# kekeliu-whu/Wildcat-SLAM

Measured on AMD Instinct MI355X. Metric: surfel-extract Mpts/s, higher is better.
Workload: dtype f64; 1 GPU; C2: 1M-pt single scan (G2 patch lattice, 999936 pts -> 31248 surfels) per GPU, voxel-grid + 3-level octree + per-cell 3x3 PCA; input = the reference's 48-byte hilti_ros::Point records, consumed in place; points_per_gpu=999936, surfels_per_gpu=31248, parallelism=sweep-per-gpu x1

## Files before the change

### wildcat-slam_amd/csrc/ctx.h

```cpp
#pragma once
#include <hip/hip_runtime.h>

#include <cstdarg>
#include <cstdio>
#include <cstdlib>
#include <cstring>
#include <string>
#include <vector>

#include "../../include/wildcat_hip.h"

struct wc_window_state;

struct wc_buf {
  void *p = nullptr;
  size_t cap = 0;
  bool pooled = false;
  bool plain = false;
};

#ifdef WC_DEV_KNOBS
#define WC_DBG(P, bit) ((P).dbg & (bit))
#else
#define WC_DBG(P, bit) 0
#endif

struct wc_dev_opts {
  int exact_sums = 0;
  int debug_skip = 0;
  int fx_merge_min = 3;
  int fx_split = -1;
  int no_bucket_sort = 0;
  int ex_sync = 0;
  int match_pair_serial = 0;
  int lm_dense = 0;
  int lm_side_stream = 1;
  int lm_one_collective = 0;
  int map_mom_pts = 1;
  int map_lin_groups = 0;
  int lm_dense_radius = 7;
  int lm_radius0 = -1;
};
inline bool wc_log_env(const char *name) { return getenv(name) != nullptr; }

struct wc_ctx {
  int device = 0;
// ... 37 lines not shown
    int general_calls = 0;
    bool bucket_attr_set = false;
    uint32_t lds_cap = 256;
    bool unordered = false;
    uint32_t last_splits = 256;
    uint32_t ticket = 0, ticket_seq = 0;
    bool fx_active = false;
    bool fx_dirty = false;
    uint32_t fx_last_flags = 0, fx_fallbacks = 0, fx_last_why = 0;
    bool fx_spill_full = false;
    bool fx_split = false;
    bool batch_defer = false, deferred = false;
    unsigned fx_tiles = 0, fx_ngrid = 0;
    bool fx_long_lists = false;
    bool fx_long_lists2 = false;
    uint32_t fx_backoff = 0, fx_skip_calls = 0;
    bool fx_ctrl_ready = false;
    int fx_parity = 0;
    bool precleared = false;
    bool layer2_done = true;
    int (*tail)(wc_ctx *, bool) = nullptr;
    alignas(16) unsigned char roots_args[768];
    uint64_t total_slots;
    uint32_t bin_cap;
    unsigned slot_end_bit;
    bool fast_slots;
  } ex;
  wc_window_state *win = nullptr;
  wc_ctx *aux = nullptr;
  hipEvent_t ev_aux = nullptr;
// ... 74 lines not shown
```

### wildcat-slam_amd/csrc/ctx.hip

```cpp
#include "ctx.h"

#include <cmath>
#include <cstring>
#include <mutex>

extern "C" const char *wc_version(void) { return "wildcat_hip 0.1 (gfx950)"; }

extern "C" int wc_device_count(void) {
  int n = 0;
  if (hipGetDeviceCount(&n) != hipSuccess) return 0;
  return n;
}

extern "C" void wc_params_default(wc_params *p) {
  std::memset(p, 0, sizeof(*p));
  p->voxel_size = 0.8f;
  p->max_layer = 2;
  p->min_points = 20;
  p->planer_threshold = 0.01f;
  p->min_plane_likeness = 0.1;
  p->cluster_gap = 0.05;
  p->cluster_min_points = 20;
  p->center_scale = 1.0;
  p->angular_scale = 5.0 * M_PI / 180.0;
// ... 22 lines not shown
  if (p->knn_k < 1 || p->knn_k > 16) return wc_fail(ctx, WC_ERR_ARG, "knn_k must be 1..16");
  return WC_OK;
}

namespace {
struct DevOpt {
  const char *name, *env;
  int wc_dev_opts::*field;
  bool flag_only;
};
const DevOpt kDevOpts[] = {
    {"exact_sums", "WC_EXACT_SUMS", &wc_dev_opts::exact_sums, true},
    {"debug_skip", "WC_DEBUG_SKIP", &wc_dev_opts::debug_skip, false},
    {"fx_merge_min", "WC_FX_MERGE_MIN", &wc_dev_opts::fx_merge_min, false},
    {"fx_split", "WC_FX_SPLIT", &wc_dev_opts::fx_split, false},
    {"no_bucket_sort", "WC_NO_BUCKET_SORT", &wc_dev_opts::no_bucket_sort, true},
    {"ex_sync", "WC_EX_SYNC", &wc_dev_opts::ex_sync, true},
    {"match_pair_serial", "WC_MATCH_PAIR_SERIAL", &wc_dev_opts::match_pair_serial, true},
    {"lm_dense", "WC_LM_DENSE", &wc_dev_opts::lm_dense, true},
    {"lm_one_collective", "WC_LM_ONE_COLLECTIVE", &wc_dev_opts::lm_one_collective, true},
    {"lm_side_stream", "WC_LM_SIDE_STREAM", &wc_dev_opts::lm_side_stream, false},
    {"map_mom_pts", "WC_MAP_MOM_PTS", &wc_dev_opts::map_mom_pts, false},
    {"map_lin_groups", "WC_MAP_LIN_GROUPS", &wc_dev_opts::map_lin_groups, false},
    {"lm_dense_radius", "WC_LM_DENSE_RADIUS", &wc_dev_opts::lm_dense_radius, false},
    {"lm_radius0", "WC_LM_RADIUS0", &wc_dev_opts::lm_radius0, false},
};
}

namespace {
struct DevPool {
// ... 318 lines not shown
```

### wildcat-slam_amd/csrc/extract.hip

```cpp
#include <hip/hip_runtime.h>
#include <type_traits>

#include <chrono>
#include <cstdlib>
#include <cstring>
#include <rocprim/rocprim.hpp>

#include "ctx.h"
#include "dmath.h"

namespace {

constexpr int kMom = 11;
constexpr int kProdStride = 66;
constexpr unsigned kRootsGrid = 256 * 16;
constexpr unsigned kEmitGrid = 256 * 8;
constexpr unsigned kRoots2Grid = 256 * 4;
constexpr int kBuckets = 4096;
constexpr int kTile = 2048;
constexpr uint32_t kFlagKeyRange = 1u, kFlagSlotOverflow = 2u, kFlagTimeRange = 4u, kFlagBucketOverflow = 8u, kFlagSlotBinOverflow = 16u, kFlagLdsOverflow = 32u;

struct ExParams {
  double vs;
  float vs_f;
// ... 1238 lines not shown
  for (int off = 32; off >= 1; off >>= 1) part += __shfl_xor(part, off);
  if (lane == 0) s_red[w] = part;
  __syncthreads();
  uint32_t base = s_red[0] + s_red[1] + s_red[2] + s_red[3];
  const uint32_t c0 = own.x, c1 = own.y, c2 = own.z, c3 = own.w;
  if (bid == nblk - 1 && t == 0) {
    status[0] = base + c0 + c1 + c2 + c3;
    uint32_t *hm = host_mailbox(status);
    if (hm) {
      hm[0] = base + c0 + c1 + c2 + c3;
      uint32_t queued = status[4];
      const uint32_t *fxc = counts + kBuckets;
      for (int j = 0; j < 16; ++j) queued += fxc[(16 + j) * 32];
      hm[4] = queued;
      hm[5] = status[5];
    }
  }
  base += (w > 0 ? c0 : 0u) + (w > 1 ? c1 : 0u) + (w > 2 ? c2 : 0u);
  const uint32_t c = w == 0 ? c0 : (w == 1 ? c1 : (w == 2 ? c2 : c3));
  if (c == 0) return;
  if (c > bin_cap) {
    if (lane == 0) raise_flag(status, kFlagSlotBinOverflow);
    return;
  }
  auto before = [&](uint64_t other, uint64_t mine) -> bool {
    if ((other >> 32) == (mine >> 32) && other != mine) {
      const double to = slots[(uint32_t)other].t, tm = slots[(uint32_t)mine].t;
      return to < tm || (to == tm && surfel_id_less(slot_ids[(uint32_t)other], slot_ids[(uint32_t)mine]));
    }
    return other < mine;
// ... 333 lines not shown
}

template <typename K>
int sort_pairs(wc_ctx *ctx, K *kin, K *kout, uint32_t *vin, uint32_t *vout, size_t n, unsigned end_bit) {
  using cfg = rocprim::radix_sort_config<rocprim::default_config, rocprim::default_config, rocprim::default_config, 0>;
  size_t tmp = 0;
  WC_HIP(ctx, rocprim::radix_sort_pairs<cfg>(nullptr, tmp, kin, kout, vin, vout, n, 0u, end_bit, ctx->stream));
  WC_TRY(wc_ensure(ctx, ctx->b_sorttmp, tmp));
  tmp = ctx->b_sorttmp.cap;
  WC_HIP(ctx, rocprim::radix_sort_pairs<cfg>(ctx->b_sorttmp.p, tmp, kin, kout, vin, vout, n, 0u, end_bit, ctx->stream));
  return WC_OK;
}

#include "extract_fast.inc"
#include "extract_split.inc"

int fx_ensure_zero(wc_ctx *ctx, wc_buf &b, size_t bytes) {
  if (bytes <= b.cap) return WC_OK;
  WC_TRY(wc_ensure(ctx, b, bytes));
  WC_HIP(ctx, hipMemsetAsync(b.p, 0, b.cap, ctx->stream));
  return WC_OK;
}

bool fx_applicable(const wc_ctx *ctx, uint64_t n, double t_lo, double t_hi) {
  const wc_params &P = ctx->P;
  if (P.exact_sums || ctx->dev.exact_sums) return false;
  if (n < 64 || !(P.voxel_size > 0.0f) || P.voxel_size >= 0.99f) return false;
  if (!(P.cluster_gap > 1e-6) || !(t_hi > t_lo)) return false;
  if ((t_hi - t_lo) / (P.cluster_gap * 0.999) >= 1048000.0) return false;
  return true;
// ... 28 lines not shown
  A.inv_vs = 1.0 / (double)P.voxel_size;
  A.qs = 4294967296.0, A.inv_q = 1.0 / 4294967296.0, A.inv_qq = std::ldexp(1.0, -44);
  uint32_t mr = 1024;
  while ((uint64_t)mr * 8 < n) mr *= 2;
  A.mr_per = mr / kFxSub, A.mq_per = std::max(64u, mr / 2 / kFxSub);
  uint32_t tr = 2048;
  while ((uint64_t)tr * 4 < n) tr *= 2;
  A.tr_mask = tr - 1;
  A.static_map = n <= 2000000ull ? 1u : 0u;
  {
    const uintptr_t px = (uintptr_t)pts.xyz, pt = (uintptr_t)pts.time;
    if (pts.xyz_stride == 48u && pts.time_stride == 48u && pt == px + 24u && px % 16u == 0u)
      A.fmt = 1u;
    else if (pts.xyz_stride == 12u && pts.time_stride == 8u && px % 16u == 0u && pt % 16u == 0u)
      A.fmt = 2u;
  }
  const unsigned tiles = (unsigned)((n + kFxTile - 1) / kFxTile);
  A.rec_tiles = tiles;
  const uint64_t spill_full = ((uint64_t)tiles + 7) / 8 * kFxTile;
  A.spill_per = (uint32_t)((n <= 8000000ull || ctx->ex.fx_spill_full) ? spill_full : std::max<uint64_t>(1024, n / 32));
  A.rec_cap = tiles * (uint32_t)kFxRecTile + 8u * A.spill_per;
  const uint64_t total_slots = std::max<uint64_t>((n * (uint64_t)(P.max_layer + 1)) / (uint64_t)P.cluster_min_points + 1, (uint64_t)kFxSub * 256);
  uint32_t bin_cap = 64;
  while (bin_cap < kSlotBinMax && (uint64_t)bin_cap * kBuckets < 2 * total_slots) bin_cap *= 2;
  WC_TRY(fx_ensure_zero(ctx, ctx->b_fx[0], (size_t)tr * 4));
  WC_TRY(wc_ensure(ctx, ctx->b_fx[1], (size_t)mr * 4));
  WC_TRY(fx_ensure_zero(ctx, ctx->b_fx[2], (size_t)tr * kFxBlockW * 8));
  WC_TRY(fx_ensure_zero(ctx, ctx->b_fx[3], (size_t)A.mq_per * kFxSub * kFxBlockW * 8));
  WC_TRY(wc_ensure(ctx, ctx->b_fx[4], (size_t)2 * A.rec_cap * kFxRecW * 8));
  const unsigned ngrid = std::min<unsigned>(256 * 16, std::max<unsigned>(64, (unsigned)(n / 256)));
// ... 59 lines not shown
  };
  if (dbg) fprintf(stderr, "[fx] n=%llu tiles=%u mr_per=%u mq_per=%u tr=%u slots_per=%u bin_cap=%u\n", (unsigned long long)n, tiles, A.mr_per, A.mq_per, tr, A.slots_per, bin_cap);
  if (ctx->ex.batch_defer) {
    static_assert(sizeof(FxArgs) <= sizeof(ctx->ex.roots_args), "ctx.h: roots_args too small");
    std::memcpy(ctx->ex.roots_args, &A, sizeof(A));
    ctx->ex.total_slots = total_slots;
    ctx->ex.bin_cap = bin_cap;
    ctx->ex.fast_slots = true;
    ctx->ex.tail = &fx_tail;
    ctx->ex.d_out = d_out, ctx->ex.d_ids = d_ids, ctx->ex.cap = cap;
    ctx->ex.layer2_done = P.max_layer >= 2 && ctx->ex.last_splits > 0;
    ctx->ex.fx_tiles = tiles, ctx->ex.fx_ngrid = std::max(64u, ngrid / 8u);
    ctx->ex.deferred = true;
    return WC_OK;
  }
  k_fx_acc<1><<<tiles, kFxThreads, 0, st>>>(A);
  dbg_sync("k_fx_acc<1>");
  mark(2);
  if (ctx->ex.fx_long_lists) k_fx_merge<1><<<std::min<unsigned>(ngrid * 2u, 8192u), 128, 0, st>>>(A);
  if (ctx->ex.fx_split) {
    k_fx_walk<1><<<ngrid, 64, 0, st>>>(A);
    dbg_sync("k_fx_walk<1>");
    k_fx_test<1><<<ngrid, 64, 0, st>>>(A);
  } else {
    k_fx_nodes<1><<<ngrid, 64, 0, st>>>(A);
  }
  dbg_sync("k_fx_nodes<1>");
  mark(3);
  static_assert(sizeof(FxArgs) <= sizeof(ctx->ex.roots_args), "ctx.h: roots_args too small");
  std::memcpy(ctx->ex.roots_args, &A, sizeof(A));
  ctx->ex.total_slots = total_slots;
// ... 6 lines not shown

constexpr int kMailTicket = 120;
__global__ void k_ex_ticket(uint32_t *host_word, uint32_t ticket) {
  __hip_atomic_store(host_word, ticket, __ATOMIC_RELEASE, __HIP_MEMORY_SCOPE_SYSTEM);
}

int fx_tail(wc_ctx *ctx, bool layer2) {
  hipStream_t st = ctx->stream;
  FxArgs A;
  std::memcpy(&A, ctx->ex.roots_args, sizeof(A));
  auto mark = [&](int i) {
    if (ctx->ex_prof && (ctx->ex_prof_mode != 2 || i == 1 || i == 5)) (void)hipEventRecord(ctx->ex_ev[i], st);
  };
  if (layer2) {
    const unsigned tiles = (unsigned)((A.pts.n + kFxTile - 1) / kFxTile);
    k_fx_acc<2><<<tiles, kFxThreads, 0, st>>>(A);
    const unsigned ngrid = std::min<unsigned>(256 * 16, std::max<unsigned>(64, (unsigned)(A.pts.n / 256)));
    if (ctx->ex.fx_long_lists2) k_fx_merge<2><<<std::min(8192u, std::max(64u, ctx->ex.last_splits)), 128, 0, st>>>(A);
    const unsigned g2 = std::min(std::min(256u * 8u, ngrid), std::max(64u, ctx->ex.last_splits));
    if (ctx->ex.fx_split) {
      k_fx_walk<2><<<g2, 64, 0, st>>>(A);
      k_fx_test<2><<<g2, 64, 0, st>>>(A);
    } else {
      k_fx_nodes<2><<<g2, 64, 0, st>>>(A);
    }
  }
  ctx->ex.layer2_done = layer2;
  mark(4);
  uint32_t *next_ctrl = (uint32_t *)ctx->b_fx[5].p + (size_t)(ctx->ex.fx_parity ^ 1) * kCtrlWords;
  static_assert(kCtrlWords <= (kBuckets / 4) * 256, "k_slot_emit's grid covers the control block");
  k_slot_emit<<<kBuckets / 4, 256, 0, st>>>(A.slot_counts, A.slot_bins, ctx->ex.bin_cap, (const wc_surfel *)ctx->b_slots.p,
// ... 291 lines not shown
      for (int i = 0; i < 24; ++i)
        if (ctx->h_status[32 + i]) ctx->ex.fx_last_why |= 1u << i;
      if (ctx->ex.fx_last_why & (1u << 4)) ctx->ex.fx_spill_full = true;
      ctx->ex.fx_backoff = std::min(32u, std::max(1u, ctx->ex.fx_backoff * 2u));
      ctx->ex.fx_skip_calls = ctx->ex.fx_backoff - 1u;
      ctx->ex.fx_dirty = true;
      ctx->ex.fx_ctrl_ready = false;
      ctx->ex.fx_active = false;
      ctx->ex.general = ctx->ex.general_calls > 0;
      WC_TRY(run_pipeline<uint32_t>(ctx, ctx->ex.pts, ctx->ex.t_lo, ctx->ex.t_hi, ctx->ex.d_out, ctx->ex.d_ids, ctx->ex.cap, !ctx->ex.general, true));
      WC_TRY(wait());
    } else {
      const uint32_t n_fast = ctx->h_status[0];
      ctx->ex.fx_long_lists = ctx->h_status[15] != 0u;
      ctx->ex.fx_long_lists2 = ctx->h_status[16] != 0u;
      if (h_n_out) *h_n_out = n_fast;
      ctx->ex.fx_parity ^= 1;
      ctx->ex.fx_backoff = 0;
      if (n_fast > ctx->ex.cap)
        return wc_fail(ctx, WC_ERR_CAPACITY, "output capacity %llu < %u surfels", (unsigned long long)ctx->ex.cap, n_fast);
      return WC_OK;
    }
  }
  while ((ctx->h_status[1] & kFlagLdsOverflow) && !(ctx->h_status[1] & (kFlagBucketOverflow | kFlagKeyRange)) && !ctx->ex.general &&
         ctx->ex.lds_cap < kPtBinMax) {
    ctx->ex.lds_cap *= 2;
    WC_TRY(run_pipeline<uint32_t>(ctx, ctx->ex.pts, ctx->ex.t_lo, ctx->ex.t_hi, ctx->ex.d_out, ctx->ex.d_ids, ctx->ex.cap, true, true));
    WC_TRY(wait());
  }
  if ((ctx->h_status[1] & kFlagLdsOverflow) && !ctx->ex.general) ctx->h_status[1] |= kFlagBucketOverflow;
// ... 54 lines not shown
  hipStream_t st = ctx->stream;
  std::vector<FxArgs> args;
  std::vector<SlotEmitArgs> emit;
  std::vector<uint32_t> s_acc(1, 0u), s_nodes(1, 0u), s_g2(1, 0u), flags;
  bool any_l2 = false, any_merge = false;
  for (int k = 0; k < K; ++k) {
    wc_ctx *sub = ctx->batch_subs[k];
    if (sub->stream != st) WC_TRY(wc_ctx_set_stream(sub, st));
    if (std::memcmp(&sub->P, &ctx->P, sizeof(wc_params)) != 0) WC_TRY(wc_ctx_set_params(sub, &ctx->P));
    if (std::memcmp(&sub->dev, &ctx->dev, sizeof(wc_dev_opts)) != 0) {
      sub->dev = ctx->dev;
      sub->ex.fx_backoff = sub->ex.fx_skip_calls = 0;
    }
    sub->ex.batch_defer = true;
    sub->ex.deferred = false;
    const int rc = wc_extract_surfels_enqueue(sub, &jobs[k].pts, jobs[k].t_lo, jobs[k].t_hi, jobs[k].d_out, jobs[k].d_ids, jobs[k].cap);
    sub->ex.batch_defer = false;
    if (rc != WC_OK) {
      for (int j = 0; j <= k; ++j) {
        wc_ctx *pj = ctx->batch_subs[j];
        if (pj->ex.deferred || j == k) pj->ex.fx_dirty = true, pj->ex.active = false, pj->ex.deferred = false;
      }
      return wc_fail(ctx, rc, "wc_extract_surfels_batch (sweep %d): %s", k, wc_last_error(sub));
    }
    if (!sub->ex.deferred) continue;
    FxArgs A;
    std::memcpy(&A, sub->ex.roots_args, sizeof(A));
    args.push_back(A);
    const uint32_t g2 = std::min(std::min(256u * 8u, sub->ex.fx_ngrid), std::max(64u, sub->ex.last_splits));
    s_acc.push_back(s_acc.back() + sub->ex.fx_tiles);
// ... 15 lines not shown
  std::memcpy(host.data(), args.data(), sizeof(FxArgs) * Kd);
  std::memcpy(host.data() + o_emit, emit.data(), sizeof(SlotEmitArgs) * Kd);
  uint32_t *tab = (uint32_t *)(host.data() + o_tab);
  std::memcpy(tab, s_acc.data(), (Kd + 1) * 4);
  std::memcpy(tab + (Kd + 1), s_nodes.data(), (Kd + 1) * 4);
  std::memcpy(tab + 2 * (Kd + 1), s_g2.data(), (Kd + 1) * 4);
  std::memcpy(tab + 3 * (Kd + 1), flags.data(), Kd * 4);
  WC_TRY(wc_ensure(ctx, ctx->b_batch, bytes));
  WC_HIP(ctx, hipMemcpyAsync(ctx->b_batch.p, host.data(), bytes, hipMemcpyHostToDevice, st));
  WC_HIP(ctx, hipStreamSynchronize(st));
  const unsigned char *d = (const unsigned char *)ctx->b_batch.p;
  const uint32_t *dt = (const uint32_t *)(d + o_tab);
  FxBatch B;
  B.args = (const FxArgs *)d, B.K = Kd, B.flags = dt + 3 * (Kd + 1);
  B.start = dt;
  k_fx_acc_b<1><<<s_acc.back(), kFxThreads, 0, st>>>(B);
  B.start = dt + (Kd + 1);
  if (any_merge) k_fx_merge_b<1><<<s_nodes.back(), 128, 0, st>>>(B);
  k_fx_walk_b<1><<<s_nodes.back(), 64, 0, st>>>(B);
  k_fx_test_b<1><<<s_nodes.back(), 64, 0, st>>>(B);
  if (any_l2) {
    B.start = dt;
    k_fx_acc_b<2><<<s_acc.back(), kFxThreads, 0, st>>>(B);
    B.start = dt + 2 * (Kd + 1);
    if (any_merge) k_fx_merge_b<2><<<s_g2.back(), 128, 0, st>>>(B);
    k_fx_walk_b<2><<<s_g2.back(), 64, 0, st>>>(B);
    k_fx_test_b<2><<<s_g2.back(), 64, 0, st>>>(B);
  }
  k_slot_emit_b<<<(unsigned)Kd * (kBuckets / 4), 256, 0, st>>>((const SlotEmitArgs *)(d + o_emit), Kd);
  WC_HIP(ctx, hipGetLastError());
  return WC_OK;
}

extern "C" int wc_extract_surfels_batch_finish(wc_ctx *ctx, uint64_t *h_n_out, int K) {
  wc_dev_guard dg_(ctx);
  if (!ctx || !h_n_out || K < 1 || K > (int)ctx->batch_subs.size()) return wc_fail(ctx, WC_ERR_ARG, "%s: null or out-of-range argument", __func__);
  int first_rc = WC_OK;
  for (int k = 0; k < K; ++k) {
// ... 21 lines not shown
  if (!ctx || !h_ms5 || !ctx->ex_ev[0]) return wc_fail(ctx, WC_ERR_ARG, "%s: null or out-of-range argument", __func__);
  WC_HIP(ctx, hipEventSynchronize(ctx->ex_ev[5]));
  if (ctx->ex_prof_mode == 2) {
    for (int i = 0; i < 5; ++i) h_ms5[i] = 0.f;
    WC_HIP(ctx, hipEventElapsedTime(&h_ms5[1], ctx->ex_ev[1], ctx->ex_ev[5]));
    return WC_OK;
  }
  for (int i = 0; i < 5; ++i) WC_HIP(ctx, hipEventElapsedTime(&h_ms5[i], ctx->ex_ev[i], ctx->ex_ev[i + 1]));
  return WC_OK;
}

extern "C" int wc_debug_status(wc_ctx *ctx, uint32_t *h_out64) {
  wc_dev_guard dg_(ctx);
  if (!ctx || !h_out64) return wc_fail(ctx, WC_ERR_ARG, "%s: null or out-of-range argument", __func__);
  for (int i = 0; i < 64; ++i) h_out64[i] = i < 16 ? ctx->h_status[i] : 0u;
  h_out64[59] = ctx->ex.fx_long_lists ? 1u : 0u;
  h_out64[60] = ctx->ex.fx_fallbacks;
  h_out64[61] = ctx->ex.fx_active ? 1u : 0u;
  h_out64[62] = ctx->ex.fx_last_flags;
  h_out64[63] = ctx->ex.fx_last_why;
#ifdef WC_PROF_ROOTS
  const size_t nslots = ctx->ex.pts.n / (size_t)(ctx->P.min_points + 1) + 1;
  std::vector<uint32_t> rows(nslots * 8);
  WC_HIP(ctx, hipMemcpy(rows.data(), ctx->b_misc[6].p, nslots * 32, hipMemcpyDeviceToHost));
  double sum[8] = {0};
  uint32_t cnt = 0;
  for (size_t r = 0; r < nslots; ++r)
    if (rows[r * 8 + 1]) {
      ++cnt;
      for (int i = 0; i < 8; ++i) sum[i] += rows[r * 8 + i];
// ... 47 lines not shown
```

### wildcat-slam_amd/csrc/extract_fast.inc

```

constexpr uint32_t kFlagFxFallback = 64u;
constexpr int kFxPts = 4;
constexpr int kFxThreads = 256;
constexpr int kFxTile = kFxPts * kFxThreads;
constexpr int kFxLds = 256;
constexpr int kFxLdsProbe = 12;
constexpr int kFxDirect = 16;
constexpr int kFxRecTile = kFxLds + (kFxThreads / 64) * 4 * kFxDirect;
constexpr int kFxSlots = 16;
constexpr int kFxRecW = 16;
constexpr int kFxHdrW = 16;
constexpr int kFxBlockW = kFxHdrW + 8 * kFxSlots / 2;
constexpr int kFxSub = 16;
constexpr uint32_t kFxStRoots = 0, kFxStNodes2 = 1, kFxStSlots = 2, kFxStSpillBank = 3;
constexpr int kFxCntStride = 32;
constexpr int kFxCntWords = 4 * kFxSub * kFxCntStride;
constexpr unsigned long long kFxTMax = 0xFFFFFFFFFFFFull;
constexpr double kFxMagic = 6755399441055744.0, kFxMagic2 = 7083549724304467820544.0;
constexpr unsigned long long kFxMagicBits = 0x4338000000000000ull;
constexpr uint32_t kFxMagicHi = 0x43380000u, kFxMagic2Hi = 0x44780000u;

struct FxArgs {
  wc_points pts;
  ExParams P;
// ... 3 lines not shown
  double inv_span;
  double inv_vs;
  double qs, inv_q, inv_qq;
  uint32_t *rkey;
  uint32_t *rlist;
  uint32_t tr_mask;
  uint32_t static_map;
  unsigned long long *blk;
  unsigned long long *blk2;
  unsigned long long *rec;
  uint32_t rec_tiles;
  uint32_t spill_per;
  uint32_t rec_cap;
  uint32_t mr_per, mq_per;
  uint32_t fmt;
  uint32_t *status;
  uint32_t *cnt;
  unsigned long long *jobs;
  unsigned long long *nodes;
  uint32_t *wdesc;
  unsigned long long *jobpool;
  uint32_t jobpool_per;
  wc_surfel *slots;
  wc_surfel_id *slot_ids;
  uint32_t slots_per;
  uint32_t *slot_counts;
  uint64_t *slot_bins;
  uint32_t slot_bin_cap;
};

// ... 9 lines not shown
  k *= 0x7FEB352Du;
  k ^= k >> 15;
  k *= 0x846CA68Bu;
  k ^= k >> 16;
  return k;
}

__device__ __forceinline__ int fx_vox(double p, double vs, double inv_vs) {
  const double q = p * inv_vs;
  const double r = rint(q);
  if (fabs(q - r) > 1e-9 * (fabs(r) + 1.0)) return (int)floor(q);
  return (int)floor(p / vs);
}

constexpr int kFxStMaxProbe = 20;
__device__ __forceinline__ uint32_t fx_root_slot(const FxArgs &A, uint32_t key1, uint32_t sub, bool insert, uint32_t maxprobe = 0u) {
  uint32_t slot = fx_hash32(key1) & A.tr_mask;
  for (int probe = 0; probe < 64; ++probe) {
    uint32_t k;
    if (insert) {
      k = atomicCAS(&A.rkey[slot], 0u, key1);
      if (k == 0u) {
        if (probe) atomicMax(&A.status[kFxStMaxProbe], (uint32_t)probe);
        const uint32_t local = atomicAdd(fx_cnt(A, kFxStRoots, sub), 1u);
        if (local < A.mr_per)
          A.rlist[sub * A.mr_per + local] = slot;
        else
          fx_fallback(A.status, 0);
        return slot;
      }
// ... 151 lines not shown
  FxRaw r;
  const uint64_t tb = (uint64_t)bid * kFxTile, n = A.pts.n;
#pragma unroll
  for (int it = 0; it < kFxPts; ++it) {
    const uint64_t i = tb + (uint64_t)it * kFxThreads + threadIdx.x;
    r.x[it] = r.y[it] = r.z[it] = 0.f, r.t[it] = 0.0;
    if (i < n) {
      const float *f = (const float *)((const char *)A.pts.xyz + i * A.pts.xyz_stride);
      r.x[it] = f[0], r.y[it] = f[1], r.z[it] = f[2];
      r.t[it] = load_t(A.pts, i);
    }
  }
  return r;
}

template <int LEVEL>
__device__ __forceinline__ void fx_acc_body(const FxArgs &A, const uint32_t bid) {
  __shared__ unsigned long long lds_raw[kFxLds * 14];
  unsigned long long *h_key = lds_raw;
  unsigned long long(*h_rec)[13] = (unsigned long long(*)[13])(lds_raw + kFxLds);
  static_assert(kFxLds * 14 * 8 >= kFxTile * 20, "staging area fits the hash area");
  const int tid = threadIdx.x;
  const ExParams &P = A.P;
  const uint32_t sub = bid & (kFxSub - 1);
  const uint64_t n = A.pts.n;
  const uint64_t base = ((uint64_t)bid * kFxThreads + tid) * kFxPts;
  static_assert(kFxPts == 4, "the LDS transposition reads four points per lane");
  const bool direct = A.fmt == 2u && ((uint64_t)bid + 1u) * kFxTile <= n;
  FxRaw raw;
  float4 da = make_float4(0.f, 0.f, 0.f, 0.f), db = da, dc = da;
  double2 dt01 = make_double2(0.0, 0.0), dt23 = dt01;
  if (direct) {
    const float4 *xp = (const float4 *)((const char *)A.pts.xyz + base * 12u);
    const double2 *tp = (const double2 *)((const char *)A.pts.time + base * 8u);
    da = xp[0], db = xp[1], dc = xp[2];
    dt01 = tp[0], dt23 = tp[1];
  } else {
    raw = fx_acc_load(A, bid);
  }
  double x0, y0, z0;
  load_xyz(A.pts, 0, x0, y0, z0);
  const int k0x = fx_vox(x0, P.vs, A.inv_vs), k0y = fx_vox(y0, P.vs, A.inv_vs), k0z = fx_vox(z0, P.vs, A.inv_vs);
  const float q0 = P.vs_f / 4;

  double px[kFxPts], py[kFxPts], pz[kFxPts], pt[kFxPts];
  if (direct) {
    const float4 a = da, b = db, c = dc;
    const double2 t01 = dt01, t23 = dt23;
    for (int i = tid; i < kFxLds * 14; i += kFxThreads) lds_raw[i] = 0ull;
    px[0] = a.x, py[0] = a.y, pz[0] = a.z, px[1] = a.w, py[1] = b.x, pz[1] = b.y;
    px[2] = b.z, py[2] = b.w, pz[2] = c.x, px[3] = c.y, py[3] = c.z, pz[3] = c.w;
    pt[0] = t01.x, pt[1] = t01.y, pt[2] = t23.x, pt[3] = t23.y;
    __syncthreads();
  } else {
    double *s_t = (double *)lds_raw;
    float *s_x = (float *)(s_t + kFxTile), *s_y = s_x + kFxTile, *s_z = s_y + kFxTile;
#pragma unroll
    for (int it = 0; it < kFxPts; ++it) {
      s_x[it * kFxThreads + tid] = raw.x[it], s_y[it * kFxThreads + tid] = raw.y[it], s_z[it * kFxThreads + tid] = raw.z[it];
      s_t[it * kFxThreads + tid] = raw.t[it];
    }
    __syncthreads();
    {
      const float4 vx = ((const float4 *)s_x)[tid], vy = ((const float4 *)s_y)[tid], vz = ((const float4 *)s_z)[tid];
      const double2 t01 = ((const double2 *)s_t)[2 * tid], t23 = ((const double2 *)s_t)[2 * tid + 1];
      px[0] = vx.x, px[1] = vx.y, px[2] = vx.z, px[3] = vx.w;
      py[0] = vy.x, py[1] = vy.y, py[2] = vy.z, py[3] = vy.w;
      pz[0] = vz.x, pz[1] = vz.y, pz[2] = vz.z, pz[3] = vz.w;
      pt[0] = t01.x, pt[1] = t01.y, pt[2] = t23.x, pt[3] = t23.y;
    }
    __syncthreads();
    for (int i = tid; i < kFxLds * 14; i += kFxThreads) lds_raw[i] = 0ull;
    __syncthreads();
  }
  if (WC_DBG(P, 4)) {
    double sacc = 0;
#pragma unroll
    for (int j = 0; j < kFxPts; ++j) sacc += px[j] + py[j] + pz[j] + pt[j];
    if (sacc == 1.2345) h_key[tid] = 1ull;
    return;
  }
  auto flush_lds = [&](unsigned long long code, const FxPart &a) -> bool {
    uint32_t s = fx_hash32((uint32_t)code ^ (uint32_t)(code >> 29)) & (kFxLds - 1);
    for (int probe = 0; probe < kFxLdsProbe; ++probe) {
      const unsigned long long old = atomicCAS(&h_key[s], 0ull, code);
      if (old == 0ull || old == code) {
        fx_add_cell(&h_rec[s][0], a);
        return true;
      }
      s = (s + 1) & (kFxLds - 1);
    }
    return false;
  };

  unsigned long long code[kFxPts];
  double tmag[kFxPts];
  uint32_t qlx[kFxPts], qly[kFxPts], qlz[kFxPts];
  bool bad_key = false, bad_time = false;
  int kxs[kFxPts], kys[kFxPts], kzs[kFxPts];
  {
    bool near = false;
#pragma unroll
    for (int j = 0; j < kFxPts; ++j) {
      const double qx = px[j] * A.inv_vs, qy = py[j] * A.inv_vs, qz = pz[j] * A.inv_vs;
      const double fx = floor(qx), fy = floor(qy), fz = floor(qz);
      const double dx = qx - fx, dy = qy - fy, dz = qz - fz;
      near = near || !(dx > 1e-6 && dx < 1.0 - 1e-6) || !(dy > 1e-6 && dy < 1.0 - 1e-6) || !(dz > 1e-6 && dz < 1.0 - 1e-6);
      kxs[j] = (int)fx, kys[j] = (int)fy, kzs[j] = (int)fz;
    }
    if (__ballot(near)) {
#pragma unroll
      for (int j = 0; j < kFxPts; ++j) kxs[j] = fx_vox(px[j], P.vs, A.inv_vs), kys[j] = fx_vox(py[j], P.vs, A.inv_vs), kzs[j] = fx_vox(pz[j], P.vs, A.inv_vs);
    }
  }
  uint32_t split4[kFxPts], base4[kFxPts];
  if (LEVEL == 2) {
    uint32_t key1[kFxPts], slot4[kFxPts], found4[kFxPts];
    bool ok4[kFxPts];
#pragma unroll
    for (int j = 0; j < kFxPts; ++j) {
      const int rx = kxs[j] - k0x + 512, ry = kys[j] - k0y + 512, rz = kzs[j] - k0z + 512;
      ok4[j] = base + j < n && (unsigned)rx < 1024u && (unsigned)ry < 1024u && (unsigned)rz < 1024u;
      key1[j] = ((uint32_t)rx | ((uint32_t)ry << 10) | ((uint32_t)rz << 20)) + 1u;
      slot4[j] = fx_hash32(key1[j]) & A.tr_mask;
    }
#pragma unroll
    for (int j = 0; j < kFxPts; ++j) found4[j] = ok4[j] ? __hip_atomic_load(&A.rkey[slot4[j]], __ATOMIC_RELAXED, __HIP_MEMORY_SCOPE_AGENT) : 0u;
    const uint32_t maxprobe = A.status[kFxStMaxProbe];
    bool coll = false;
#pragma unroll
    for (int j = 0; j < kFxPts; ++j) coll = coll || (ok4[j] && found4[j] != key1[j] && (found4[j] != 0u || maxprobe != 0u));
    if (__ballot(coll)) {
#pragma unroll
      for (int j = 0; j < kFxPts; ++j)
        if (ok4[j] && found4[j] != key1[j] && (found4[j] != 0u || maxprobe != 0u)) {
          const uint32_t r = fx_root_slot(A, key1[j], 0u, false, maxprobe);
          slot4[j] = r != 0xFFFFFFFFu ? r : 0u;
          found4[j] = r != 0xFFFFFFFFu ? key1[j] : 0u;
        }
    }
#pragma unroll
    for (int j = 0; j < kFxPts; ++j) {
      const bool present = ok4[j] && found4[j] == key1[j];
      const uint32_t *h32 = (const uint32_t *)(A.blk + (size_t)(present ? slot4[j] : 0u) * kFxBlockW);
      const uint2 sb = *(const uint2 *)(h32 + 12);
      split4[j] = present ? sb.x : 0u, base4[j] = present ? sb.y : 0u;
    }
  }
#pragma unroll
  for (int j = 0; j < kFxPts; ++j) {
    const bool have = base + j < n;
    const double x = px[j], y = py[j], z = pz[j], t = pt[j];
    const int kx = kxs[j], ky = kys[j], kz = kzs[j];
    const int rx = kx - k0x + 512, ry = ky - k0y + 512, rz = kz - k0z + 512;
    const bool key_ok = (unsigned)rx < 1024u && (unsigned)ry < 1024u && (unsigned)rz < 1024u;
    const uint32_t key = (uint32_t)rx | ((uint32_t)ry << 10) | ((uint32_t)rz << 20);
    const double cx = fma((double)kx, (double)P.vs_f, 0.5 * (double)P.vs_f), cy = fma((double)ky, (double)P.vs_f, 0.5 * (double)P.vs_f),
                 cz = fma((double)kz, (double)P.vs_f, 0.5 * (double)P.vs_f);
    const int bx = x > cx, by = y > cy, bz = z > cz;
    const uint32_t o1 = (uint32_t)(4 * bx + 2 * by + bz);
    const double trel = t - A.t_lo;
    const double tm = fma(trel, A.tick, kFxMagic);
    const bool time_ok = tm >= kFxMagic && tm < kFxMagic + 2199023255552.0;
    bad_key = bad_key || (have && !key_ok);
    bad_time = bad_time || (have && key_ok && !time_ok);
    bool use = have && key_ok && time_ok;
// ... 45 lines not shown
  const int lane = tid & 63, wave = tid >> 6;
  const unsigned long long lt_mask = (1ull << lane) - 1ull;
  bool bnd[kFxPts];
  {
    unsigned long long open = 0ull;
#pragma unroll
    for (int j = 0; j < kFxPts; ++j) {
      bnd[j] = code[j] != 0ull && open != 0ull && code[j] != open;
      if (code[j] != 0ull) open = code[j];
    }
  }
  const uint32_t rec0 = bid * (uint32_t)kFxRecTile + (uint32_t)kFxLds + (uint32_t)wave * 4u * (uint32_t)kFxDirect;
  auto close_partial = [&](int cls, bool closing, unsigned long long c, const FxPart &a) {
    const unsigned long long mclass = __ballot(closing);
    if (!mclass || (WC_DBG(P, 2))) return;
    if (__popcll(mclass) <= kFxDirect) {
      fx_push<LEVEL>(A, closing, c & 0x7FFFFFFFFFFFFFFFull, a, sub, rec0 + (uint32_t)cls * (uint32_t)kFxDirect + (uint32_t)__popcll(mclass & lt_mask), cls == 3 ? early : no_early);
    } else {
      const bool failed = closing && !flush_lds(c, a);
      const unsigned long long mf = __ballot(failed);
      if (mf) {
        const uint32_t sp = bid & 7u;
        uint32_t b0 = 0;
        if (lane == 0) b0 = atomicAdd(fx_cnt(A, kFxStSpillBank, sp), (uint32_t)__popcll(mf));
        b0 = (uint32_t)__shfl((int)b0, 0);
        const uint32_t k = b0 + (uint32_t)__popcll(mf & lt_mask);
        const bool room = k < A.spill_per;
        if (failed && !room) fx_fallback(A.status, 4);
        fx_push<LEVEL>(A, failed && room, c & 0x7FFFFFFFFFFFFFFFull, a, sub, A.rec_tiles * (uint32_t)kFxRecTile + sp * A.spill_per + k, no_early);
      }
    }
// ... 122 lines not shown
    const uint32_t list_base = (uint32_t)__shfl((int)e_base, __ffsll((long long)e_cm) - 1);
    if (e_made) {
      const uint32_t local = list_base + (uint32_t)__popcll(e_cm & ((1ull << l) - 1ull));
      if (local < A.mr_per)
        A.rlist[sub * A.mr_per + local] = early.s0;
      else
        fx_fallback(A.status, 5);
    }
  }
}

template <int LEVEL>
__global__ void __launch_bounds__(kFxThreads) k_fx_acc(FxArgs A) {
  fx_acc_body<LEVEL>(A, blockIdx.x);
}

struct FxBatch {
  const FxArgs *args;
  const uint32_t *start;
  const uint32_t *flags;
  int K;
};
__device__ __forceinline__ int fx_batch_find(const FxBatch &B, uint32_t b, uint32_t &local) {
  int k = 0;
  while (k + 1 < B.K && b >= B.start[k + 1]) ++k;
  local = b - B.start[k];
  return k;
}
#define WC_FX_BATCH_ARGS(sA, B, k)                                                                 \
  __shared__ FxArgs sA;                                                                            \
  static_assert(sizeof(FxArgs) % 8 == 0, "copied as 64-bit words");                                 \
  for (uint32_t w_ = threadIdx.x; w_ < sizeof(FxArgs) / 8; w_ += blockDim.x)                      \
    ((unsigned long long *)&sA)[w_] = ((const unsigned long long *)&(B).args[k])[w_];              \
  __syncthreads();
template <int LEVEL>
__global__ void __launch_bounds__(kFxThreads) k_fx_acc_b(FxBatch B) {
  uint32_t bid;
  const int k = fx_batch_find(B, blockIdx.x, bid);
  if (LEVEL == 2 && !(B.flags[k] & 1u)) return;
  WC_FX_BATCH_ARGS(sA, B, k)
  fx_acc_body<LEVEL>(sA, bid);
}

template <int LEVEL>
__device__ __forceinline__ void fx_merge_body(const FxArgs &A, const uint32_t bid, const uint32_t nblk) {
  const uint32_t bank = LEVEL == 1 ? kFxStRoots : kFxStNodes2;
  const uint32_t per = LEVEL == 1 ? A.mr_per : A.mq_per;
  uint32_t total = 0, cnts[kFxSub];
#pragma unroll
  for (int j = 0; j < kFxSub; ++j) {
    cnts[j] = min(*fx_cnt(A, bank, j), per);
    total += cnts[j];
  }
  for (uint32_t gi = bid; gi < total; gi += nblk) {
    uint32_t pidx = 0, rem = gi;
    bool found = false;
// ... 743 lines not shown
```

### wildcat-slam_amd/python/wildcat_slam_amd/lib.py

```python
import ctypes as C
import os
import re
import weakref

import numpy as np

from . import records as R

_CSRC = os.path.join(os.path.dirname(os.path.dirname(os.path.dirname(os.path.abspath(__file__)))), "csrc")
_SO = os.path.join(_CSRC, "libwildcat_hip.so")
_INCLUDE = os.path.join(os.path.dirname(os.path.dirname(_CSRC)), "include")
_LIB = None

WC_OK, WC_ERR_CAPACITY = 0, 1


class WildcatError(RuntimeError):
    def __init__(self, code, msg):
        super().__init__(f"wildcat_hip error {code}: {msg}")
        self.code = code


def so_path():
    return _SO
# ... 204 lines not shown
        def finish():
            rc = f_fin(h, n_ref)
            if rc:
                ck(rc)
            return n.value

        return enqueue, finish

    def set_exact_sums(self, exact):
        self.params.exact_sums = 1 if exact else 0
        self.set_params(self.params)

    def extract_path_info(self):
        w = (C.c_uint32 * 64)()
        self._ck(self.lib.wc_debug_status(self.h, w))
        return dict(fast=bool(w[61]), fallbacks=int(w[60]), flags=int(w[62]), why=int(w[63]), long_lists=bool(w[59]))

    def extract_profile(self, enable=True):
        self._ck(self.lib.wc_extract_profile(self.h, C.c_int(int(enable))))

    def extract_stage_ms(self):
        ms = (C.c_float * 5)()
        self._ck(self.lib.wc_extract_stage_ms(self.h, ms))
        return dict(zip(("init", "point_sort", "roots_stream", "roots_emit", "slot_order"), [float(v) for v in ms]))

    def extract_surfels(self, points, hint=True, cap=None):
        n = len(points)
        assert points.dtype.itemsize == 48, "POINT records are 48 bytes (np.concatenate packs the dtype: use synth.concat_points)"
        cap = cap or max(1024, (3 * n) // 20 + 1)
        d_pts = self.to_device(points) if n else self.alloc(48)
        d_out, d_ids = self.alloc(cap * 144), self.alloc(cap * 16)
# ... 648 lines not shown
```

Before: 21050 Mpts/s.

## Adaptively pick a strided point-to-lane assignment in the fast accumulation kernel

```diff
diff --git a/profiles/dev/sim_stride.py b/profiles/dev/sim_stride.py
--- /dev/null
+++ b/profiles/dev/sim_stride.py
@@ -0,0 +1,33 @@
+import os
+import sys
+
+import numpy as np
+
+sys.path.insert(0, os.path.join(os.path.dirname(os.path.abspath(__file__)), "..", "..", "wildcat-slam_amd", "python"))
+from wildcat_slam_amd import synth
+
+TILE, STRIDES = 1024, (1, 16, 32, 64, 128)
+
+
+def closed_per_point(pts, gap=0.05):
+    n = len(pts) // TILE * TILE
+    xyz = np.stack([pts["x"], pts["y"], pts["z"]], -1).astype(np.float64)[:n]
+    half = np.floor(xyz / (synth.VS / 2)).astype(np.int64)
+    tbin = np.floor((pts["time"][:n] - pts["time"][0]) / (gap * 0.999)).astype(np.int64)
+    _, code = np.unique(np.concatenate([half, tbin[:, None]], 1), axis=0, return_inverse=True)
+    code = code.reshape(-1, TILE)
+    cells = np.mean([len(np.unique(row)) for row in code])
+    out = []
+    for s in STRIDES:
+        p = np.arange(TILE)
+        c = code[:, (p % (TILE // s)) * s + p // (TILE // s)]
+        ends = np.ones(c.shape, bool)
+        ends[:, :-1] = c[:, :-1] != c[:, 1:]
+        ends[:, 63::64] = True
+        out.append(ends.mean())
+    return out, cells
+
+
+for name, pts in (("g1_room (firing order, 32 beams)", synth.g1_room(1_000_000, seed=synth.SEED + 3)), ("g2 C2", synth.g2_lattice(3906)[0])):
+    frac, cells = closed_per_point(pts)
+    print("%-34s" % name, " ".join("S=%d: %.3f" % (s, f) for s, f in zip(STRIDES, frac)), " cells per tile: %.0f" % cells)
diff --git a/wildcat-slam_amd/csrc/ctx.h b/wildcat-slam_amd/csrc/ctx.h
--- a/wildcat-slam_amd/csrc/ctx.h
+++ b/wildcat-slam_amd/csrc/ctx.h
@@ -30,6 +30,7 @@
   int debug_skip = 0;
   int fx_merge_min = 3;
   int fx_split = -1;
+  int fx_lane_stride = -1;
   int no_bucket_sort = 0;
   int ex_sync = 0;
   int match_pair_serial = 0;
@@ -97,6 +98,8 @@
     unsigned fx_tiles = 0, fx_ngrid = 0;
     bool fx_long_lists = false;
     bool fx_long_lists2 = false;
+    uint32_t fx_stride = 1;
+    uint32_t fx_stride_used = 1;
     uint32_t fx_backoff = 0, fx_skip_calls = 0;
     bool fx_ctrl_ready = false;
     int fx_parity = 0;
diff --git a/wildcat-slam_amd/csrc/ctx.hip b/wildcat-slam_amd/csrc/ctx.hip
--- a/wildcat-slam_amd/csrc/ctx.hip
+++ b/wildcat-slam_amd/csrc/ctx.hip
@@ -60,6 +60,7 @@
     {"debug_skip", "WC_DEBUG_SKIP", &wc_dev_opts::debug_skip, false},
     {"fx_merge_min", "WC_FX_MERGE_MIN", &wc_dev_opts::fx_merge_min, false},
     {"fx_split", "WC_FX_SPLIT", &wc_dev_opts::fx_split, false},
+    {"fx_lane_stride", "WC_FX_LANE_STRIDE", &wc_dev_opts::fx_lane_stride, false},
     {"no_bucket_sort", "WC_NO_BUCKET_SORT", &wc_dev_opts::no_bucket_sort, true},
     {"ex_sync", "WC_EX_SYNC", &wc_dev_opts::ex_sync, true},
     {"match_pair_serial", "WC_MATCH_PAIR_SERIAL", &wc_dev_opts::match_pair_serial, true},
diff --git a/wildcat-slam_amd/csrc/extract.hip b/wildcat-slam_amd/csrc/extract.hip
--- a/wildcat-slam_amd/csrc/extract.hip
+++ b/wildcat-slam_amd/csrc/extract.hip
@@ -1276,6 +1276,7 @@
       for (int j = 0; j < 16; ++j) queued += fxc[(16 + j) * 32];
       hm[4] = queued;
       hm[5] = status[5];
+      for (int j = 0; j < 5; ++j) hm[20 + j] = status[24 + j];
     }
   }
   base += (w > 0 ? c0 : 0u) + (w > 1 ? c1 : 0u) + (w > 2 ? c2 : 0u);
@@ -1639,6 +1640,7 @@
 
 #include "extract_fast.inc"
 #include "extract_split.inc"
+static_assert(kFxStFit == 24 && kFxMailFit == 20 && kFxFitCand == 5, "k_slot_emit mails status words 24 .. 28 as mailbox words 20 .. 24");
 
 int fx_ensure_zero(wc_ctx *ctx, wc_buf &b, size_t bytes) {
   if (bytes <= b.cap) return WC_OK;
@@ -1697,6 +1699,11 @@
       A.fmt = 1u;
     else if (pts.xyz_stride == 12u && pts.time_stride == 8u && px % 16u == 0u && pt % 16u == 0u)
       A.fmt = 2u;
+  }
+  {
+    const int pin = ctx->dev.fx_lane_stride;
+    A.lane_stride = (pin == 1 || pin == 16 || pin == 32 || pin == 64 || pin == 128) ? (uint32_t)pin : ctx->ex.fx_stride;
+    ctx->ex.fx_stride_used = A.lane_stride;
   }
   const unsigned tiles = (unsigned)((n + kFxTile - 1) / kFxTile);
   A.rec_tiles = tiles;
@@ -1786,7 +1793,10 @@
     ctx->ex.deferred = true;
     return WC_OK;
   }
-  k_fx_acc<1><<<tiles, kFxThreads, 0, st>>>(A);
+  if (A.lane_stride > 1u)
+    k_fx_acc_s<1><<<tiles, kFxThreads, 0, st>>>(A);
+  else
+    k_fx_acc<1><<<tiles, kFxThreads, 0, st>>>(A);
   dbg_sync("k_fx_acc<1>");
   mark(2);
   if (ctx->ex.fx_long_lists) k_fx_merge<1><<<std::min<unsigned>(ngrid * 2u, 8192u), 128, 0, st>>>(A);
@@ -1823,7 +1833,10 @@
   };
   if (layer2) {
     const unsigned tiles = (unsigned)((A.pts.n + kFxTile - 1) / kFxTile);
-    k_fx_acc<2><<<tiles, kFxThreads, 0, st>>>(A);
+    if (A.lane_stride > 1u)
+      k_fx_acc_s<2><<<tiles, kFxThreads, 0, st>>>(A);
+    else
+      k_fx_acc<2><<<tiles, kFxThreads, 0, st>>>(A);
     const unsigned ngrid = std::min<unsigned>(256 * 16, std::max<unsigned>(64, (unsigned)(A.pts.n / 256)));
     if (ctx->ex.fx_long_lists2) k_fx_merge<2><<<std::min(8192u, std::max(64u, ctx->ex.last_splits)), 128, 0, st>>>(A);
     const unsigned g2 = std::min(std::min(256u * 8u, ngrid), std::max(64u, ctx->ex.last_splits));
@@ -2145,6 +2158,13 @@
       const uint32_t n_fast = ctx->h_status[0];
       ctx->ex.fx_long_lists = ctx->h_status[15] != 0u;
       ctx->ex.fx_long_lists2 = ctx->h_status[16] != 0u;
+      {
+        static const uint32_t cand[kFxFitCand] = {1u, 16u, 32u, 64u, 128u};
+        int best = 0;
+        for (int k = 1; k < kFxFitCand; ++k)
+          if (ctx->h_status[kFxMailFit + k] > ctx->h_status[kFxMailFit + best]) best = k;
+        ctx->ex.fx_stride = cand[best];
+      }
       if (h_n_out) *h_n_out = n_fast;
       ctx->ex.fx_parity ^= 1;
       ctx->ex.fx_backoff = 0;
@@ -2229,6 +2249,7 @@
     }
     sub->ex.batch_defer = true;
     sub->ex.deferred = false;
+    sub->ex.fx_stride = ctx->ex.fx_stride;
     const int rc = wc_extract_surfels_enqueue(sub, &jobs[k].pts, jobs[k].t_lo, jobs[k].t_hi, jobs[k].d_out, jobs[k].d_ids, jobs[k].cap);
     sub->ex.batch_defer = false;
     if (rc != WC_OK) {
@@ -2274,14 +2295,21 @@
   FxBatch B;
   B.args = (const FxArgs *)d, B.K = Kd, B.flags = dt + 3 * (Kd + 1);
   B.start = dt;
-  k_fx_acc_b<1><<<s_acc.back(), kFxThreads, 0, st>>>(B);
+  const bool strided = args[0].lane_stride > 1u;
+  if (strided)
+    k_fx_acc_sb<1><<<s_acc.back(), kFxThreads, 0, st>>>(B);
+  else
+    k_fx_acc_b<1><<<s_acc.back(), kFxThreads, 0, st>>>(B);
   B.start = dt + (Kd + 1);
   if (any_merge) k_fx_merge_b<1><<<s_nodes.back(), 128, 0, st>>>(B);
   k_fx_walk_b<1><<<s_nodes.back(), 64, 0, st>>>(B);
   k_fx_test_b<1><<<s_nodes.back(), 64, 0, st>>>(B);
   if (any_l2) {
     B.start = dt;
-    k_fx_acc_b<2><<<s_acc.back(), kFxThreads, 0, st>>>(B);
+    if (strided)
+      k_fx_acc_sb<2><<<s_acc.back(), kFxThreads, 0, st>>>(B);
+    else
+      k_fx_acc_b<2><<<s_acc.back(), kFxThreads, 0, st>>>(B);
     B.start = dt + 2 * (Kd + 1);
     if (any_merge) k_fx_merge_b<2><<<s_g2.back(), 128, 0, st>>>(B);
     k_fx_walk_b<2><<<s_g2.back(), 64, 0, st>>>(B);
@@ -2333,6 +2361,7 @@
   wc_dev_guard dg_(ctx);
   if (!ctx || !h_out64) return wc_fail(ctx, WC_ERR_ARG, "%s: null or out-of-range argument", __func__);
   for (int i = 0; i < 64; ++i) h_out64[i] = i < 16 ? ctx->h_status[i] : 0u;
+  h_out64[58] = ctx->ex.fx_stride_used;
   h_out64[59] = ctx->ex.fx_long_lists ? 1u : 0u;
   h_out64[60] = ctx->ex.fx_fallbacks;
   h_out64[61] = ctx->ex.fx_active ? 1u : 0u;
diff --git a/wildcat-slam_amd/csrc/extract_fast.inc b/wildcat-slam_amd/csrc/extract_fast.inc
--- a/wildcat-slam_amd/csrc/extract_fast.inc
+++ b/wildcat-slam_amd/csrc/extract_fast.inc
@@ -41,6 +41,8 @@
   uint32_t rec_cap;
   uint32_t mr_per, mq_per;
   uint32_t fmt;
+  uint32_t lane_stride;
+  uint32_t spare_;
   uint32_t *status;
   uint32_t *cnt;
   unsigned long long *jobs;
@@ -80,6 +82,7 @@
 }
 
 constexpr int kFxStMaxProbe = 20;
+constexpr int kFxStFit = 24, kFxMailFit = 20, kFxFitCand = 5;
 __device__ __forceinline__ uint32_t fx_root_slot(const FxArgs &A, uint32_t key1, uint32_t sub, bool insert, uint32_t maxprobe = 0u) {
   uint32_t slot = fx_hash32(key1) & A.tr_mask;
   for (int probe = 0; probe < 64; ++probe) {
@@ -261,19 +264,29 @@
   return r;
 }
 
-template <int LEVEL>
+template <int LEVEL, bool STR = false>
 __device__ __forceinline__ void fx_acc_body(const FxArgs &A, const uint32_t bid) {
   __shared__ unsigned long long lds_raw[kFxLds * 14];
   unsigned long long *h_key = lds_raw;
   unsigned long long(*h_rec)[13] = (unsigned long long(*)[13])(lds_raw + kFxLds);
   static_assert(kFxLds * 14 * 8 >= kFxTile * 20, "staging area fits the hash area");
+  constexpr int kStage = STR ? kFxTile + kFxTile / 32 : kFxTile;
+  constexpr int kProxW = (kFxTile + kFxTile / 32) * 20 / 4;
+  static_assert((kProxW + kFxTile + 4 * kFxFitCand) * 4 <= kFxLds * 14 * 8, "proxies and counts fit behind the staging area");
   const int tid = threadIdx.x;
   const ExParams &P = A.P;
   const uint32_t sub = bid & (kFxSub - 1);
   const uint64_t n = A.pts.n;
   const uint64_t base = ((uint64_t)bid * kFxThreads + tid) * kFxPts;
   static_assert(kFxPts == 4, "the LDS transposition reads four points per lane");
-  const bool direct = A.fmt == 2u && ((uint64_t)bid + 1u) * kFxTile <= n;
+  const bool fit = LEVEL == 1 && (bid & 63u) == 0u;
+  const bool direct = !STR && !fit && A.fmt == 2u && ((uint64_t)bid + 1u) * kFxTile <= n;
+  uint32_t li0 = (uint32_t)tid * kFxPts, lstep = 1u;
+  if (STR) {
+    const uint32_t ls = (uint32_t)__ffs((int)A.lane_stride) - 1u;
+    li0 = ((li0 & ((kFxTile >> ls) - 1u)) << ls) + (li0 >> (10u - ls));
+    lstep = A.lane_stride;
+  }
   FxRaw raw;
   float4 da = make_float4(0.f, 0.f, 0.f, 0.f), db = da, dc = da;
   double2 dt01 = make_double2(0.0, 0.0), dt23 = dt01;
@@ -301,20 +314,54 @@
     __syncthreads();
   } else {
     double *s_t = (double *)lds_raw;
-    float *s_x = (float *)(s_t + kFxTile), *s_y = s_x + kFxTile, *s_z = s_y + kFxTile;
+    float *s_x = (float *)(s_t + kStage), *s_y = s_x + kStage, *s_z = s_y + kStage;
+    uint32_t *s_prox = (uint32_t *)lds_raw + kProxW, *s_fit = s_prox + kFxTile;
+    auto sidx = [](uint32_t i) -> uint32_t { return STR ? i + (i >> 5) : i; };
 #pragma unroll
     for (int it = 0; it < kFxPts; ++it) {
-      s_x[it * kFxThreads + tid] = raw.x[it], s_y[it * kFxThreads + tid] = raw.y[it], s_z[it * kFxThreads + tid] = raw.z[it];
-      s_t[it * kFxThreads + tid] = raw.t[it];
+      const uint32_t i = sidx((uint32_t)(it * kFxThreads + tid));
+      s_x[i] = raw.x[it], s_y[i] = raw.y[it], s_z[i] = raw.z[it];
+      s_t[i] = raw.t[it];
+    }
+    if (fit) {
+      const float hv = (float)(2.0 * A.inv_vs);
+#pragma unroll
+      for (int it = 0; it < kFxPts; ++it) {
+        const int hx = (int)floorf(raw.x[it] * hv), hy = (int)floorf(raw.y[it] * hv), hz = (int)floorf(raw.z[it] * hv);
+        s_prox[it * kFxThreads + tid] = ((uint32_t)hx & 0x7FFu) | (((uint32_t)hy & 0x7FFu) << 11) | (((uint32_t)hz & 0x3FFu) << 22);
+      }
     }
     __syncthreads();
-    {
+    if (STR) {
+#pragma unroll
+      for (int j = 0; j < kFxPts; ++j) {
+        const uint32_t i = sidx(li0 + (uint32_t)j * lstep);
+        px[j] = s_x[i], py[j] = s_y[i], pz[j] = s_z[i], pt[j] = s_t[i];
+      }
+    } else {
       const float4 vx = ((const float4 *)s_x)[tid], vy = ((const float4 *)s_y)[tid], vz = ((const float4 *)s_z)[tid];
       const double2 t01 = ((const double2 *)s_t)[2 * tid], t23 = ((const double2 *)s_t)[2 * tid + 1];
       px[0] = vx.x, px[1] = vx.y, px[2] = vx.z, px[3] = vx.w;
       py[0] = vy.x, py[1] = vy.y, py[2] = vy.z, py[3] = vy.w;
       pz[0] = vz.x, pz[1] = vz.y, pz[2] = vz.z, pz[3] = vz.w;
       pt[0] = t01.x, pt[1] = t01.y, pt[2] = t23.x, pt[3] = t23.y;
+    }
+    if (fit) {
+      const uint32_t nt = (uint32_t)min((uint64_t)kFxTile, n - (uint64_t)bid * kFxTile);
+      uint32_t c01 = 0u, c23 = 0u, c4 = 0u;
+#pragma unroll
+      for (int it = 0; it < kFxPts; ++it) {
+        const uint32_t i = (uint32_t)(it * kFxThreads + tid), p = s_prox[i];
+        auto same = [&](uint32_t S) -> uint32_t { return i + S < nt && s_prox[i + S] == p ? 1u : 0u; };
+        c01 += same(1u) | (same(16u) << 16), c23 += same(32u) | (same(64u) << 16), c4 += same(128u);
+      }
+      for (int m = 1; m < 64; m <<= 1) c01 += (uint32_t)__shfl_xor((int)c01, m), c23 += (uint32_t)__shfl_xor((int)c23, m), c4 += (uint32_t)__shfl_xor((int)c4, m);
+      if ((tid & 63) == 0) {
+        uint32_t *f = s_fit + (tid >> 6) * kFxFitCand;
+        f[0] = c01 & 0xFFFFu, f[1] = c01 >> 16, f[2] = c23 & 0xFFFFu, f[3] = c23 >> 16, f[4] = c4;
+      }
+      __syncthreads();
+      if (tid < kFxFitCand) atomicAdd(&A.status[kFxStFit + tid], s_fit[tid] + s_fit[kFxFitCand + tid] + s_fit[2 * kFxFitCand + tid] + s_fit[3 * kFxFitCand + tid]);
     }
     __syncthreads();
     for (int i = tid; i < kFxLds * 14; i += kFxThreads) lds_raw[i] = 0ull;
@@ -340,6 +387,9 @@
     return false;
   };
 
+  bool have4[kFxPts];
+#pragma unroll
+  for (int j = 0; j < kFxPts; ++j) have4[j] = STR ? (uint64_t)bid * kFxTile + li0 + (uint32_t)j * lstep < n : base + j < n;
   unsigned long long code[kFxPts];
   double tmag[kFxPts];
   uint32_t qlx[kFxPts], qly[kFxPts], qlz[kFxPts];
@@ -367,7 +417,7 @@
 #pragma unroll
     for (int j = 0; j < kFxPts; ++j) {
       const int rx = kxs[j] - k0x + 512, ry = kys[j] - k0y + 512, rz = kzs[j] - k0z + 512;
-      ok4[j] = base + j < n && (unsigned)rx < 1024u && (unsigned)ry < 1024u && (unsigned)rz < 1024u;
+      ok4[j] = have4[j] && (unsigned)rx < 1024u && (unsigned)ry < 1024u && (unsigned)rz < 1024u;
       key1[j] = ((uint32_t)rx | ((uint32_t)ry << 10) | ((uint32_t)rz << 20)) + 1u;
       slot4[j] = fx_hash32(key1[j]) & A.tr_mask;
     }
@@ -396,7 +446,7 @@
   }
 #pragma unroll
   for (int j = 0; j < kFxPts; ++j) {
-    const bool have = base + j < n;
+    const bool have = have4[j];
     const double x = px[j], y = py[j], z = pz[j], t = pt[j];
     const int kx = kxs[j], ky = kys[j], kz = kzs[j];
     const int rx = kx - k0x + 512, ry = ky - k0y + 512, rz = kz - k0z + 512;
@@ -472,7 +522,7 @@
   auto close_partial = [&](int cls, bool closing, unsigned long long c, const FxPart &a) {
     const unsigned long long mclass = __ballot(closing);
     if (!mclass || (WC_DBG(P, 2))) return;
-    if (__popcll(mclass) <= kFxDirect) {
+    if (!STR && __popcll(mclass) <= kFxDirect) {
       fx_push<LEVEL>(A, closing, c & 0x7FFFFFFFFFFFFFFFull, a, sub, rec0 + (uint32_t)cls * (uint32_t)kFxDirect + (uint32_t)__popcll(mclass & lt_mask), cls == 3 ? early : no_early);
     } else {
       const bool failed = closing && !flush_lds(c, a);
@@ -625,6 +675,10 @@
 __global__ void __launch_bounds__(kFxThreads) k_fx_acc(FxArgs A) {
   fx_acc_body<LEVEL>(A, blockIdx.x);
 }
+template <int LEVEL>
+__global__ void __launch_bounds__(kFxThreads) k_fx_acc_s(FxArgs A) {
+  fx_acc_body<LEVEL, true>(A, blockIdx.x);
+}
 
 struct FxBatch {
   const FxArgs *args;
@@ -651,6 +705,14 @@
   if (LEVEL == 2 && !(B.flags[k] & 1u)) return;
   WC_FX_BATCH_ARGS(sA, B, k)
   fx_acc_body<LEVEL>(sA, bid);
+}
+template <int LEVEL>
+__global__ void __launch_bounds__(kFxThreads) k_fx_acc_sb(FxBatch B) {
+  uint32_t bid;
+  const int k = fx_batch_find(B, blockIdx.x, bid);
+  if (LEVEL == 2 && !(B.flags[k] & 1u)) return;
+  WC_FX_BATCH_ARGS(sA, B, k)
+  fx_acc_body<LEVEL, true>(sA, bid);
 }
 
 template <int LEVEL>
diff --git a/wildcat-slam_amd/python/wildcat_slam_amd/lib.py b/wildcat-slam_amd/python/wildcat_slam_amd/lib.py
--- a/wildcat-slam_amd/python/wildcat_slam_amd/lib.py
+++ b/wildcat-slam_amd/python/wildcat_slam_amd/lib.py
@@ -242,7 +242,7 @@
     def extract_path_info(self):
         w = (C.c_uint32 * 64)()
         self._ck(self.lib.wc_debug_status(self.h, w))
-        return dict(fast=bool(w[61]), fallbacks=int(w[60]), flags=int(w[62]), why=int(w[63]), long_lists=bool(w[59]))
+        return dict(fast=bool(w[61]), fallbacks=int(w[60]), flags=int(w[62]), why=int(w[63]), long_lists=bool(w[59]), lane_stride=int(w[58]))
 
     def extract_profile(self, enable=True):
         self._ck(self.lib.wc_extract_profile(self.h, C.c_int(int(enable))))
```

Result: slower. 20510 Mpts/s (-2.6%).
